# jaak-s/libfastsparse

Measured on AMD Instinct MI355X. Metric: fp64 CSR SpMV effective GB/s (% HBM3E peak), higher is better.
Workload: dtype f64

## Files before the change

### libfastsparse_amd/csrc/fs_common.h

```cpp
#pragma once

#include <hip/hip_runtime.h>
#include <stdint.h>
#include <stdio.h>
#include <mutex>
#include <string>
#include <vector>

#include "fastsparse_hip.h"
#include "fs_geometry.h"

namespace fs {

constexpr int kBlock = 256;
constexpr int kChunk = 2048;
constexpr int kPerThread = kChunk / kBlock;

void set_error(const std::string &msg);
int hip_fail(hipError_t e, const char *what, const char *file, int line);

#define FS_HIP(call)                                                   \
  do {                                                                 \
    hipError_t e_ = (call);                                            \
    if (e_ != hipSuccess) return ::fs::hip_fail(e_, #call, __FILE__, __LINE__); \
// ... 25 lines not shown
  int nrow = 0, ncol = 0;
  int64_t nnz = 0;
  int *row_ptr = nullptr;
  int *cols = nullptr;
  double *vals = nullptr;
  bool owns = true;
  bool released = false, released_valued = false;
  bool has_vals() const { return vals != nullptr || (released && released_valued); }
  int nchunks = 0;
  int *first_row = nullptr;
  double *head = nullptr;
  double *tail = nullptr;
  int spanning = 0;
  TiledCsr *tiled = nullptr;
  TiledCsr *tiledx = nullptr;
  BinnedCsr *binned = nullptr;
  BinnedCsr *binned2 = nullptr, *binned4 = nullptr;
  bool tried2 = false, tried4 = false;
  double *spmm_scratch = nullptr;
  size_t spmm_scratch_doubles = 0;
  signed char spmm_choice[17] = {};
  float candidate_ms[4] = {0.f, 0.f, 0.f, 0.f};
  mutable int max_row_len = -1;
  bool two_pass_clear_win = false;
  float build_ms[8] = {0.f, 0.f, 0.f, 0.f, 0.f, 0.f, 0.f, 0.f};
  struct PartCuts { int n = 0, kind = 0; bool cut = false; std::vector<int> rows, units; };
  std::vector<PartCuts> part_plans;
  PartCuts partk[2];
};

struct TiledCsr {
  bool built = false;
  bool ldsx = false;
  int R = 0, W = 0, P = 0, J = 0, lcol_bits = kTiledColBits;
  float entries_per_tile = 0.f;
  unsigned *pk = nullptr;
  double *vals = nullptr;
  int4 *items = nullptr;
  int *item_ptr = nullptr;
  int nitems = 0;
  int *panel_row = nullptr;
  int split = 0;
  int nvrow = 0;
  int *vfirst = nullptr;
  double *yv = nullptr;
  int slots = 256;
  HostMirror<int> h_panel_row, h_chunk_panel;
  std::vector<int> h_chunk_need;
  int nchunks = 0;
  int *chunk_panel = nullptr;
  int *chunk_item = nullptr;
  bool shared = false;
  bool orderable = false;
  int *chunk_ord = nullptr;
  int *ticket = nullptr;
};


struct LongRows {
  int nlong = 0;
  int64_t n = 0;
  int bcols = kLongBandA;
  int B = 0;
  int *row = nullptr;
  uint16_t *lcol = nullptr;
  uint16_t *lrow = nullptr;
  double *vals = nullptr;
  int64_t *band_ptr = nullptr;
  unsigned *seg_ptr = nullptr;
  double *ylong = nullptr;
  double *ypart = nullptr;
  int nwg = 0;
};

struct BinnedCsr {
  bool built = false;
  LongRows *lr = nullptr;
  int kw = 1;
  int bcols = kBinCols;
  int B = 0, P = 0;
  int64_t n = 0;
  uint16_t *lcol = nullptr;
  double *vals = nullptr;
  unsigned *gdst = nullptr;
  uint16_t *lrow = nullptr;
  uint8_t *lrow8 = nullptr;
  uint16_t *gbase = nullptr;
  int64_t dummies = 0;
  bool lrow_tried = false;
  double *prod = nullptr;
  unsigned *band_ptr = nullptr;
  int nwg1 = 0;
  int slots = 0;
  unsigned *bin_ptr = nullptr;
  int *panel_row = nullptr;
  int split = 0, nvrow = 0;
  int *vfirst = nullptr;
  double *yv = nullptr;
  HostMirror<unsigned> h_band_ptr;
  HostMirror<int> h_panel_row, h_vfirst;
};

struct HostPipe {
  double *sx = nullptr, *sy = nullptr;
  size_t cx = 0, cy = 0;
  hipStream_t stream = nullptr;
  static constexpr int kMaxChunks = 32;
  hipEvent_t ev[kMaxChunks] = {};
  int nev = 0;
};
void free_host_pipe(HostPipe &H);

}

struct fs_matrix_s {
  fs::DeviceCsr a;
  fs::DeviceCsr at;
  bool has_t = false;
  int device = 0;
  std::mutex lock;
  hipStream_t last_stream = nullptr;
  bool last_async = false;
  fs::HostPipe pipe;
};

struct fs_cbcsr_s {
  int nrow = 0, ncol = 0, nblocks = 0, colblocksize = 0;
  int64_t nnz = 0;
  int *row_ptr = nullptr;
  int *cols = nullptr;
  int device = 0;
  fs::DeviceCsr cells;
  double *cell_sums = nullptr;
  bool use_cells = false;
  fs::DeviceCsr rows;
  bool use_rows = false;
  std::mutex lock;
};

namespace fs {

bool roctx_enabled();
void roctx_push(const char *name);
void roctx_pop();
struct Range {
  bool on;
  explicit Range(const char *name) : on(roctx_enabled()) { if (on) roctx_push(name); }
  ~Range() { if (on) roctx_pop(); }
  Range(const Range &) = delete;
  Range &operator=(const Range &) = delete;
};
#define FS_RANGE(name) ::fs::Range fs_range_(name)

struct Options {
  int strict_order = 0;
  int spmv_kernel = 0;
  int tiling = 1;
  int tile_rows = 0;
  int tile_cols = 0;
  int tile_split = 0;
  int tiled_flags = 0;
  int reproducible = 0;
  int bin_wgs = 0;
  int bin_flags = 0;
  int bin_rows = 0;
  int ldsx = 1;
// ... 195 lines not shown
```

### libfastsparse_amd/csrc/fs_copies.hip

```cpp
#include <algorithm>
#include <vector>

#include "fs_format_util.h"
#include "fs_plan.h"

namespace fs {

static_assert(sizeof(WorkItem) == sizeof(int4) && sizeof(RowLen) == sizeof(int2), "fs_plan.h's plain structs are the device's int4 / int2");

__global__ void piece_count_kernel(int nrow, int split, const int *__restrict__ row_ptr, int *__restrict__ cnt)
{
  const int r = blockIdx.x * blockDim.x + threadIdx.x;
  if (r > nrow) return;
  if (r == nrow) { cnt[r] = 0; return; }
  const int len = row_ptr[r + 1] - row_ptr[r];
  cnt[r] = len <= split ? 1 : (len + split - 1) / split;
}

__global__ void vrow_fill_kernel(int nrow, int split, const int *__restrict__ row_ptr, const int *__restrict__ vfirst,
                                 int *__restrict__ vrow_ptr)
{
  const int r = blockIdx.x * blockDim.x + threadIdx.x;
  if (r > nrow) return;
  if (r == nrow) { vrow_ptr[vfirst[nrow]] = row_ptr[nrow]; return; }
// ... 636 lines not shown
  if (mode == 1 && !ldsx && tiled_hopeless(A.nnz, ntiles, P, slots, x_bytes)) return FS_OK;
  if (ntiles >= (1ll << 31)) return FS_OK;
  T->R = R; T->W = W; T->P = P; T->J = J;
  T->entries_per_tile = (float)((double)A.nnz / (double)ntiles);
  FS_HIP(traced_malloc(&T->panel_row, sizeof(int) * panel_row.size()));
  FS_HIP(hipMemcpyAsync(T->panel_row, panel_row.data(), sizeof(int) * panel_row.size(), hipMemcpyHostToDevice, s));

  const size_t n = (size_t)A.nnz;
  Scratch<int> vrows, tile_ptr;
  Scratch<unsigned> keys, skeys, idx_in, idx_out;
  Scratch<char> tmp;
  FS_HIP(vrows.alloc(n));
  FS_HIP(keys.alloc(n));
  FS_HIP(skeys.alloc(n));
  FS_HIP(idx_in.alloc(n));
  FS_HIP(idx_out.alloc(n));
  FS_HIP(tile_ptr.alloc((size_t)ntiles + 1));
  FS_HIP(traced_malloc(&T->pk, sizeof(unsigned) * (n + 8)));
  if (A.vals) FS_HIP(traced_malloc(&T->vals, sizeof(double) * (n + 8)));
  hipLaunchKernelGGL(tile_key_kernel, dim3(grid_for(A.nnz)), dim3(256), 0, s, V.nvrow, A.nnz, P, W, J, V.vrow_ptr, T->panel_row,
                     A.cols, vrows.p, keys.p);
  const unsigned *sorted_keys = nullptr, *perm = nullptr;
  if (int rc = sorted_runs(tmp, keys.p, skeys.p, idx_in.p, idx_out.p, n, ntiles, tile_ptr.p, s, &sorted_keys, &perm)) return rc;
  hipLaunchKernelGGL(tile_pack_kernel, dim3(grid_for(A.nnz)), dim3(256), 0, s, A.nnz, W, J, T->lcol_bits, sorted_keys, perm,
                     vrows.p, T->panel_row, A.cols, A.vals, T->pk, T->vals);
  FS_HIP(hipGetLastError());
  std::vector<int> tp((size_t)ntiles + 1);
  FS_HIP(hipMemcpyAsync(tp.data(), tile_ptr.p, sizeof(int) * tp.size(), hipMemcpyDeviceToHost, s));
  FS_HIP(hipStreamSynchronize(s));
  std::vector<WorkItem> items;
  std::vector<int> item_ptr;
  cut_work_items(tp, P, J, items, item_ptr);
  T->nitems = (int)items.size();
  FS_HIP(traced_malloc(&T->items, sizeof(int4) * (items.size() ? items.size() : 1)));
  FS_HIP(traced_malloc(&T->item_ptr, sizeof(int) * item_ptr.size()));
  if (!items.empty()) FS_HIP(hipMemcpy(T->items, items.data(), sizeof(int4) * items.size(), hipMemcpyHostToDevice));
  FS_HIP(hipMemcpy(T->item_ptr, item_ptr.data(), sizeof(int) * item_ptr.size(), hipMemcpyHostToDevice));
  if (ldsx && T->nitems > 0)
    if (int rc = reorder_ldsx_items(T, s)) return rc;
  if (ldsx) {
    static const bool plain = [] { const char *v = getenv("FS_LDSX_ORDER"); return v && *v == '1'; }();
    std::vector<int> chunk_panel, chunk_item, chunk_ord;
    T->shared = plan_ldsx_chunks(item_ptr, (int64_t)items.size(), P, slots, plain, chunk_panel, chunk_item, chunk_ord);
    if (int rc = upload_ldsx_chunks(T, A.nrow, chunk_panel, chunk_item, chunk_ord)) return rc;
  }
  T->built = true;
  return FS_OK;
}

int build_tiled(DeviceCsr &A, hipStream_t s) { return optional_copy(build_tiled_impl(A, s, A.tiled, false), A.tiled, free_tiled_slot); }

int build_tiledx(DeviceCsr &A, hipStream_t s) { return optional_copy(build_tiled_impl(A, s, A.tiledx, true), A.tiledx, free_tiled_slot); }

__global__ void bin_key_kernel(int nvrow, int64_t nnz, int P, int bcols, const int *__restrict__ vrow_ptr,
                               const int *__restrict__ panel_row, const int *__restrict__ cols,
                               int *__restrict__ vrows, unsigned *__restrict__ keys)
{
  const int64_t i = (int64_t)blockIdx.x * blockDim.x + threadIdx.x;
  if (i >= nnz) return;
  const int v = last_le(vrow_ptr, nvrow, i);
  vrows[i] = v;
  keys[i] = (unsigned)(cols[i] / bcols) * (unsigned)P + (unsigned)last_le(panel_row, P, v);
}

__global__ void bin_groups_kernel(int B, int P, int ge, const int *__restrict__ run_ptr, unsigned *__restrict__ g1,
                                  unsigned *__restrict__ g2, const unsigned *__restrict__ xs = nullptr)
{
  const int64_t k = (int64_t)blockIdx.x * blockDim.x + threadIdx.x;
  const int64_t nruns = (int64_t)B * P;
  if (k > nruns) return;
  if (k == nruns) { g1[k] = 0; g2[k] = 0; return; }
  const int b = (int)(k / P), p = (int)(k % P);
  const unsigned dum = xs ? xs[run_ptr[k + 1]] - xs[run_ptr[k]] : 0u;
  const unsigned g = ((unsigned)(run_ptr[k + 1] - run_ptr[k]) + dum + (unsigned)ge - 1u) / (unsigned)ge;
  g1[k] = g;
  g2[(int64_t)p * B + b] = g;
}

__global__ void bin_scatter_kernel(int64_t nnz, int B, int P, int bcols, int ge, const unsigned *__restrict__ skeys,
                                   const unsigned *__restrict__ perm, const int *__restrict__ vrows,
                                   const int *__restrict__ panel_row, const int *__restrict__ cols,
                                   const double *__restrict__ vals, const int *__restrict__ run_ptr,
                                   const unsigned *__restrict__ start1, const unsigned *__restrict__ start2,
                                   uint16_t *__restrict__ lcol, double *__restrict__ vals2, uint16_t *__restrict__ lrow)
{
  const int64_t i = (int64_t)blockIdx.x * blockDim.x + threadIdx.x;
  if (i >= nnz) return;
  const unsigned key = skeys[i], src = perm[i];
  const int b = (int)(key / (unsigned)P), p = (int)(key % (unsigned)P);
  const int64_t rank = i - run_ptr[key];
  const int64_t pos1 = (int64_t)start1[key] * ge + rank;
  const int64_t pos2 = (int64_t)start2[(int64_t)p * B + b] * ge + rank;
  lcol[pos1] = (uint16_t)(cols[src] - b * bcols);
  if (vals) vals2[pos2] = vals[src];
  lrow[pos2] = (uint16_t)(vrows[src] - panel_row[p]);
}

__global__ void bin_gap_kernel(int64_t nnz, int P, const unsigned *__restrict__ skeys, const unsigned *__restrict__ perm,
                               const int *__restrict__ vrows, const int *__restrict__ run_ptr, unsigned *__restrict__ extra)
{
  const int64_t i = (int64_t)blockIdx.x * blockDim.x + threadIdx.x;
  if (i > nnz) return;
  if (i == nnz) { extra[i] = 0; return; }
  const unsigned key = skeys[i];
  unsigned e = 0;
  if (i > run_ptr[key]) {
    const int gap = vrows[perm[i]] - vrows[perm[i - 1]];
    if (gap > 255) e = (unsigned)(gap - 1) / 255u;
  }
  extra[i] = e;
}

__global__ void bin_scatter8_kernel(int64_t nnz, int B, int P, int bcols, int ge, const unsigned *__restrict__ skeys,
                                    const unsigned *__restrict__ perm, const int *__restrict__ vrows,
                                    const int *__restrict__ panel_row, const int *__restrict__ cols,
                                    const double *__restrict__ vals, const int *__restrict__ run_ptr,
                                    const unsigned *__restrict__ xs, const unsigned *__restrict__ start1,
                                    const unsigned *__restrict__ start2, uint16_t *__restrict__ lcol, double *__restrict__ vals2,
                                    uint8_t *__restrict__ lrow8, uint16_t *__restrict__ gbase)
{
  const int64_t i = (int64_t)blockIdx.x * blockDim.x + threadIdx.x;
  if (i >= nnz) return;
  const unsigned key = skeys[i], src = perm[i];
  const int b = (int)(key / (unsigned)P), p = (int)(key % (unsigned)P);
  const int64_t first = run_ptr[key];
  const unsigned dum = xs[i + 1] - xs[i];
  const int64_t slot = (i - first) + (int64_t)(xs[i] - xs[first]) + dum;
  const int64_t base1 = (int64_t)start1[key] * ge, base2 = (int64_t)start2[(int64_t)p * B + b] * ge;
  const int row = vrows[src] - panel_row[p];
  const int prev = i > first ? vrows[perm[i - 1]] - panel_row[p] : row;
  for (unsigned m = 0; m < dum; ++m) {
    const int64_t sl = slot - dum + m;
    lrow8[base2 + sl] = 255;
    if ((sl & (ge - 1)) == 0) gbase[(base2 + sl) / ge] = (uint16_t)(prev + 255 * (int)m);
  }
  const int before = prev + 255 * (int)dum;
  lcol[base1 + slot] = (uint16_t)(cols[src] - b * bcols);
  if (vals) vals2[base2 + slot] = vals[src];
  lrow8[base2 + slot] = (uint8_t)(row - before);
  if ((slot & (ge - 1)) == 0) gbase[(base2 + slot) / ge] = (uint16_t)before;
}

__global__ void bin_gdst_kernel(int B, int P, const unsigned *__restrict__ start1, const unsigned *__restrict__ start2,
                                unsigned *__restrict__ gdst)
{
  const int64_t k = (int64_t)blockIdx.x * blockDim.x + threadIdx.x;
  if (k >= (int64_t)B * P) return;
  const int b = (int)(k / P), p = (int)(k % P);
  const unsigned a = start1[k], n = start1[k + 1] - a, d = start2[(int64_t)p * B + b];
  for (unsigned j = 0; j < n; ++j) gdst[a + j] = d + j;
}

__global__ void bin_ptr_kernel(int B, int P, const unsigned *__restrict__ start1, const unsigned *__restrict__ start2,
                               unsigned *__restrict__ band_ptr, unsigned *__restrict__ bin_ptr)
{
  const int64_t k = (int64_t)blockIdx.x * blockDim.x + threadIdx.x;
  if (k <= B) band_ptr[k] = start1[k * P];
  if (k <= P) bin_ptr[k] = start2[k * B];
}

__global__ void long_candidates_kernel(int nrow, int minlen, const int *__restrict__ row_ptr, int *__restrict__ count, int cap,
                                       int2 *__restrict__ out)
{
  const int r = blockIdx.x * blockDim.x + threadIdx.x;
  if (r >= nrow) return;
  const int len = row_ptr[r + 1] - row_ptr[r];
  if (len < minlen) return;
  const int k = atomicAdd(count, 1);
  if (k < cap) out[k] = make_int2(r, len);
}

__global__ void long_mark_kernel(int nlong, const int *__restrict__ rows, int *__restrict__ row_to_long)
{
  const int i = blockIdx.x * blockDim.x + threadIdx.x;
  if (i < nlong) row_to_long[rows[i]] = i;
}

// ... 197 lines not shown
  N->split = V.split;
  N->nvrow = V.nvrow;
  const int nvrow = V.nvrow;

  std::vector<int> vp;
  if (int rc = V.fetch(vp, s)) return rc;
  static const double fill = [] { const char *v = getenv("FS_BIN_FILL"); return v && *v ? atof(v) / 100.0 : 0.8; }();
  static const int min_panels = [] { const char *v = getenv("FS_BIN_MIN_PANELS"); return v && *v ? atoi(v) : 1; }();
  const std::vector<int> panel_row = plan_two_pass_panels(vp, nvrow, A.nnz, g.R, slots, fill, min_panels, kw);
  const int P = (int)panel_row.size() - 1;
  const int B = (A.ncol + bcols - 1) / bcols;
  const int64_t nruns = (int64_t)P * B;
  if (nruns >= (1ll << 28)) return FS_OK;
  if (o.binning == 1 && two_pass_padding_dominates(A.nnz, nruns, ge)) return FS_OK;
  N->P = P; N->B = B; N->slots = slots;
  FS_HIP(traced_malloc(&N->panel_row, sizeof(int) * panel_row.size()));
  FS_HIP(hipMemcpyAsync(N->panel_row, panel_row.data(), sizeof(int) * panel_row.size(), hipMemcpyHostToDevice, s));

  const size_t n = (size_t)A.nnz;
  Scratch<int> vrows, run_ptr;
  Scratch<unsigned> keys, skeys, idx_in, idx_out, g1, g2, start1, start2;
  Scratch<char> tmp, tmp2;
  FS_HIP(vrows.alloc(n));
  FS_HIP(keys.alloc(n));
  FS_HIP(skeys.alloc(n));
  FS_HIP(idx_in.alloc(n));
  FS_HIP(idx_out.alloc(n));
  FS_HIP(run_ptr.alloc((size_t)nruns + 1));
  FS_HIP(g1.alloc((size_t)nruns + 1));
  FS_HIP(g2.alloc((size_t)nruns + 1));
  FS_HIP(start1.alloc((size_t)nruns + 1));
  FS_HIP(start2.alloc((size_t)nruns + 1));
  FS_HIP(traced_malloc(&N->band_ptr, sizeof(unsigned) * ((size_t)B + 1)));
  FS_HIP(traced_malloc(&N->bin_ptr, sizeof(unsigned) * ((size_t)P + 1)));
  hipLaunchKernelGGL(bin_key_kernel, dim3(grid_for(A.nnz)), dim3(256), 0, s, nvrow, A.nnz, P, bcols, V.vrow_ptr, N->panel_row,
                     A.cols, vrows.p, keys.p);
  const unsigned *sorted_keys = nullptr, *perm = nullptr;
  if (int rc = sorted_runs(tmp, keys.p, skeys.p, idx_in.p, idx_out.p, n, nruns, run_ptr.p, s, &sorted_keys, &perm)) return rc;
  Scratch<unsigned> extra, xs;
  Scratch<char> tmp3;
  bool rows8 = false;
  int64_t dummies = 0;
  if (kw == 1 && bcols == kBinCols && !(o.bin_flags & 64) && A.nnz > 0) {
    FS_HIP(extra.alloc(n + 1));
    FS_HIP(xs.alloc(n + 1));
    hipLaunchKernelGGL(bin_gap_kernel, dim3(grid_for(A.nnz + 1)), dim3(256), 0, s, A.nnz, P, sorted_keys, perm, vrows.p, run_ptr.p, extra.p);
    FS_HIP(hipGetLastError());
    if (int rc = device_exclusive_scan(tmp3, extra.p, xs.p, n + 1, s)) return rc;
    unsigned total = 0;
    if (int rc = read_back(&total, (const unsigned *)xs.p + n, s)) return rc;
    dummies = total;
    rows8 = (o.bin_flags & 128) || (double)total <= 0.01 * (double)A.nnz;
  }
  hipLaunchKernelGGL(bin_groups_kernel, dim3(grid_for(nruns + 1)), dim3(256), 0, s, B, P, ge, run_ptr.p, g1.p, g2.p,
                     rows8 ? (const unsigned *)xs.p : (const unsigned *)nullptr);
  FS_HIP(hipGetLastError());
  if (int rc = device_exclusive_scan(tmp2, g1.p, start1.p, (size_t)nruns + 1, s)) return rc;
  if (int rc = device_exclusive_scan(tmp2, g2.p, start2.p, (size_t)nruns + 1, s)) return rc;
  hipLaunchKernelGGL(bin_ptr_kernel, dim3(grid_for((B > P ? B : P) + 1)), dim3(256), 0, s, B, P, start1.p, start2.p, N->band_ptr,
                     N->bin_ptr);
  FS_HIP(hipGetLastError());
  unsigned total_groups = 0;
  if (int rc = read_back(&total_groups, (const unsigned *)N->band_ptr + B, s)) return rc;
  const int64_t groups = total_groups;
  if (groups >= (1ll << 28) * (int64_t)kw) return FS_OK;
  if (groups >= (1ll << 32) - 1) return FS_OK;
  N->n = groups * ge;
  if (o.binning == 1 && kw == 1 && two_pass_hopeless(N->n, A.vals != nullptr, B, ncu, bcols, nvrow, A.ncol, A.nnz)) return FS_OK;

  const size_t np = (size_t)N->n;
  FS_HIP(traced_malloc(&N->lcol, sizeof(uint16_t) * np));
  if (rows8) {
    FS_HIP(traced_malloc(&N->lrow8, np));
    FS_HIP(traced_malloc(&N->gbase, sizeof(uint16_t) * (size_t)(groups ? groups : 1)));
    N->dummies = dummies;
  } else {
    FS_HIP(traced_malloc(&N->lrow, sizeof(uint16_t) * np));
  }
  FS_HIP(traced_malloc(&N->gdst, sizeof(unsigned) * (size_t)groups));
  FS_HIP(traced_malloc(&N->prod, sizeof(double) * np * (size_t)kw));
  if (A.vals) {
    FS_HIP(traced_malloc(&N->vals, sizeof(double) * np));
    FS_HIP(hipMemsetAsync(N->vals, 0, sizeof(double) * np, s));
  }
  FS_HIP(hipMemsetD16Async((hipDeviceptr_t)N->lcol, (unsigned short)bcols, np, s));
  if (rows8) {
    FS_HIP(hipMemsetAsync(N->lrow8, 0, np, s));
    FS_HIP(hipMemsetAsync(N->gbase, 0, sizeof(uint16_t) * (size_t)(groups ? groups : 1), s));
    hipLaunchKernelGGL(bin_scatter8_kernel, dim3(grid_for(A.nnz)), dim3(256), 0, s, A.nnz, B, P, bcols, ge, sorted_keys, perm, vrows.p,
                       N->panel_row, A.cols, A.vals, run_ptr.p, xs.p, start1.p, start2.p, N->lcol, N->vals, N->lrow8, N->gbase);
  } else {
    FS_HIP(hipMemsetAsync(N->lrow, 0, sizeof(uint16_t) * np, s));
    hipLaunchKernelGGL(bin_scatter_kernel, dim3(grid_for(A.nnz)), dim3(256), 0, s, A.nnz, B, P, bcols, ge, sorted_keys, perm, vrows.p,
                       N->panel_row, A.cols, A.vals, run_ptr.p, start1.p, start2.p, N->lcol, N->vals, N->lrow);
  }
  hipLaunchKernelGGL(bin_gdst_kernel, dim3(grid_for(nruns)), dim3(256), 0, s, B, P, start1.p, start2.p, N->gdst);
  FS_HIP(hipGetLastError());

  {
    const int64_t by_size = (N->n * kw + kBinShareMin - 1) / kBinShareMin;
    N->nwg1 = (int)(by_size < ncu ? by_size : ncu);
  }
  FS_HIP(hipStreamSynchronize(s));
  N->built = true;
  return FS_OK;
}

int build_binned(DeviceCsr &A, hipStream_t s)
{
  LongRows *lr = nullptr;
  Scratch<int> main_rp, main_cols;
  Scratch<double> main_vals;
  int64_t main_nnz = 0;
  if (split_long_rows(A, s, &lr, main_rp, main_cols, main_vals, &main_nnz) != FS_OK) {
    free_long_rows(lr);
    (void)hipGetLastError();
  }
  int rc;
  if (lr) {
    DeviceCsr M;
    M.nrow = A.nrow; M.ncol = A.ncol; M.nnz = main_nnz;
    M.row_ptr = main_rp.p; M.cols = main_cols.p; M.vals = A.vals ? main_vals.p : nullptr; M.owns = false;
    rc = build_binned_impl(M, s, A.binned, 1);
    if (rc == FS_OK && A.binned && A.binned->built) { A.binned->lr = lr; lr = nullptr; }
    M = DeviceCsr();
  } else {
    rc = build_binned_impl(A, s, A.binned, 1);
  }
  free_long_rows(lr);
  return optional_copy(rc, A.binned, free_binned_slot);
}

int build_binned_k(DeviceCsr &A, int kw, hipStream_t s)
{
  if (kw != 2 && kw != 4) return FS_ERR_ARG;
  BinnedCsr *&slot = kw == 2 ? A.binned2 : A.binned4;
  (kw == 2 ? A.tried2 : A.tried4) = true;
  return optional_copy(build_binned_impl(A, s, slot, kw), slot, free_binned_slot);
}

constexpr double kTiledBestEntriesPerMs = 152e6;

template <typename F>
static int time_product(F launch, hipStream_t s, hipEvent_t e0, hipEvent_t e1, float *median, int reps = 5)
{
  float t[5] = {1e30f, 1e30f, 1e30f, 1e30f, 1e30f};
  for (int rep = -1; rep < reps; ++rep) {
    FS_HIP(hipEventRecord(e0, s));
    if (int rc = launch()) return rc;
    FS_HIP(hipEventRecord(e1, s));
    FS_HIP(hipEventSynchronize(e1));
    float ms = 0.f;
    FS_HIP(hipEventElapsedTime(&ms, e0, e1));
    if (rep >= 0) t[rep] = ms;
  }
  std::sort(t, t + reps);
  *median = t[reps / 2];
  return FS_OK;
}

int two_pass_clear_win(DeviceCsr &A, hipStream_t s, bool *win)
{
  *win = false;
  const Options &o = options();
  if (!(A.binned && A.binned->built) || o.binning != 1 || o.tiling != 1 || A.nnz < (32ll << 20) || 8.0 * (double)A.ncol <= (double)(4 << 20)) return FS_OK;
  Scratch<double> x, y;
  if (x.alloc((size_t)A.ncol) != hipSuccess || y.alloc((size_t)A.nrow) != hipSuccess) { (void)hipGetLastError(); return FS_OK; }
  FS_HIP(hipMemsetAsync(x, 0, sizeof(double) * (size_t)A.ncol, s));
  hipEvent_t e0, e1;
  FS_HIP(hipEventCreate(&e0));
  if (hipEventCreate(&e1) != hipSuccess) { (void)hipEventDestroy(e0); return FS_OK; }
  float t = 1e30f;
  const int rc = time_product([&] { return launch_spmv_binned(A, y, x, s); }, s, e0, e1, &t, 2);
  (void)hipEventDestroy(e0);
  (void)hipEventDestroy(e1);
  if (rc != FS_OK) return rc;
  *win = (double)t <= (double)A.nnz / (A.vals ? kTiledBestEntriesPerMs : 200e6);
// ... 53 lines not shown
```

### libfastsparse_amd/csrc/fs_kernels_twopass.hip

```cpp
#include <stdlib.h>

#include "fs_kernel_util.h"

namespace fs {


template <int U, bool NTLD, bool NTST, int BC>
__device__ __forceinline__ void expand_share(double *__restrict__ xband, int ncol, int B, const unsigned *__restrict__ band_ptr,
                                             const uint16_t *__restrict__ lcol, const unsigned *__restrict__ gdst,
                                             const double *__restrict__ x, int xs, double *__restrict__ prod, unsigned g0,
                                             unsigned g1)
{
  const int t = threadIdx.x;
  if (g0 >= g1) return;
  int b;
  {
    int lo = 0, hi = B - 1;
    while (lo < hi) {
      const int mid = lo + ((hi - lo + 1) >> 1);
      if (band_ptr[mid] <= g0) lo = mid; else hi = mid - 1;
    }
    b = lo;
  }
  for (unsigned g = g0; g < g1; ++b) {
// ... 301 lines not shown
      const int w = (ncol - c0 < BC) ? ncol - c0 : BC;
      if (have != b) request(b);
      __syncthreads();
#pragma unroll
      for (int j = 0; j < BC / kBinBlock; ++j) {
        const int i = j * kBinBlock + t;
        xband[i] = (i < w) ? rn[j] : 0.0;
      }
      if (t < 8) xband[BC + t] = 0.0;
      __syncthreads();
      if (b + 1 < B && eb < e_end) request(b + 1);
      if (ORDERED) {
        const int64_t s0 = band_ptr[b] + seg_ptr[b * (kLongOwners + 1) + wave], s1 = band_ptr[b] + seg_ptr[b * (kLongOwners + 1) + wave + 1];
        const int64_t lo = s0 > e ? s0 : e, hi = s1 < eb ? s1 : eb;
        for (int64_t o0 = lo; o0 < hi; o0 += 128) {
          const int64_t o = o0 + 2 * lane;
          const bool live = o < hi;
          wave_step(o, live, live ? o : lo);
        }
      } else {
        for (int64_t o0 = e; o0 < eb; o0 += 2 * kBinBlock) {
          const int64_t o = o0 + 2 * t;
          const bool live = o < eb;
          wave_step(o, live, live ? o : e);
        }
      }
      e = eb;
    }
  }
  __syncthreads();
  if (ORDERED) {
    double *__restrict__ mine = ypart + (int64_t)blockIdx.x * nlong;
    for (int i = t; i < nlong; i += kBinBlock) mine[i] = acc[i];
  } else {
    for (int i = t; i < nlong; i += kBinBlock) {
      const double v = acc[i];
      if (v != 0.0) unsafeAtomicAdd(ylong + i, v);
    }
  }
}

__global__ __launch_bounds__(kBlock) void longrows_combine_kernel(int nlong, int nwg, const double *__restrict__ ypart, double *__restrict__ ylong)
{
  const int i = blockIdx.x * kBlock + threadIdx.x;
  if (i >= nlong) return;
  double acc = 0.0;
  for (int w = 0; w < nwg; ++w) acc += ypart[(int64_t)w * nlong + i];
  ylong[i] = acc;
}

__global__ __launch_bounds__(kBlock) void longrows_scatter_kernel(int nlong, const int *__restrict__ row, const double *__restrict__ ylong,
                                                                 double *__restrict__ y, int ys, int row0, int row1)
{
  const int i = blockIdx.x * kBlock + threadIdx.x;
  if (i >= nlong) return;
  const int r = row[i];
  if (r >= row0 && r < row1) y[(int64_t)r * ys] = 0.0 + ylong[i];
}

static int launch_longrows(const DeviceCsr &A, const LongRows &L, const double *x, int xs, hipStream_t s)
{
  const bool ordered = reproducible_now();
  if (!ordered || L.n == 0 || L.nwg == 0)
    if (int rc = launch_zero(L.ylong, sizeof(double) * (size_t)L.nlong, s)) return rc;
  if (L.n == 0 || L.nwg == 0) return FS_OK;
#define FS_LONG(V, BC, NA, ORD)                                                                                              \
  hipLaunchKernelGGL((spmv_longrows_kernel<V, BC, NA, ORD>), dim3(L.nwg), dim3(kBinBlock), 0, s, A.ncol, L.B, L.nlong, L.band_ptr, \
                     L.seg_ptr, L.lcol, L.lrow, L.vals, x, xs, L.ylong, L.ypart)
#define FS_LONG2(V, BC, NA) do { if (ordered) FS_LONG(V, BC, NA, true); else FS_LONG(V, BC, NA, false); } while (0)
  if (L.bcols == kLongBandB) { if (A.has_vals()) FS_LONG2(true, kLongBandB, kLongRowsB); else FS_LONG2(false, kLongBandB, kLongRowsB); }
  else                       { if (A.has_vals()) FS_LONG2(true, kLongBandA, kLongRowsA); else FS_LONG2(false, kLongBandA, kLongRowsA); }
#undef FS_LONG2
#undef FS_LONG
  FS_HIP(hipGetLastError());
  if (ordered) {
    hipLaunchKernelGGL(longrows_combine_kernel, dim3((unsigned)((L.nlong + kBlock - 1) / kBlock)), dim3(kBlock), 0, s, L.nlong, L.nwg, L.ypart,
                       L.ylong);
    FS_HIP(hipGetLastError());
  }
  return FS_OK;
}


template <int K, int U>
__global__ __launch_bounds__(kBinBlock) void spmm_expand_kernel(
    int ncol, int B, const unsigned *__restrict__ band_ptr, const uint16_t *__restrict__ lcol,
    const unsigned *__restrict__ gdst, const double *__restrict__ X, int xs, double *__restrict__ prod)
{
  constexpr int BC = kBinCols / K;
  constexpr int GE = kBinGroup / K;
  constexpr int LP = K / 2;
  constexpr int EPS = kBinBlock / LP;
  __shared__ __attribute__((aligned(16))) double xband[kBinCols + 8];
  const int t = threadIdx.x;
  const int le = t / LP, h = t % LP;
  const uint64_t groups = band_ptr[B];
  const unsigned g0 = (unsigned)(groups * blockIdx.x / gridDim.x), g1 = (unsigned)(groups * (blockIdx.x + 1) / gridDim.x);
  if (g0 >= g1) return;
  int b;
  {
    int lo = 0, hi = B - 1;
    while (lo < hi) {
      const int mid = lo + ((hi - lo + 1) >> 1);
      if (band_ptr[mid] <= g0) lo = mid; else hi = mid - 1;
    }
    b = lo;
  }
  for (unsigned g = g0; g < g1; ++b) {
    const unsigned gb = band_ptr[b + 1] < g1 ? band_ptr[b + 1] : g1;
    if (gb <= g) continue;
    const int c0 = b * BC;
    const int w = (ncol - c0 < BC) ? ncol - c0 : BC;
    __syncthreads();
    {
      double r[kBinCols / kBinBlock];
#pragma unroll
      for (int j = 0; j < kBinCols / kBinBlock; ++j) {
        const int f = j * kBinBlock + t, i = f / K, q = f % K;
        r[j] = __builtin_nontemporal_load(X + (int64_t)(c0 + (i < w ? i : w - 1)) * xs + q);
      }
#pragma unroll
      for (int j = 0; j < kBinCols / kBinBlock; ++j) {
        const int f = j * kBinBlock + t;
        xband[f] = (f / K < w) ? r[j] : 0.0;
      }
      if (t < 8) xband[kBinCols + t] = 0.0;
    }
    __syncthreads();
    const int64_t e0 = (int64_t)g * GE, e1 = (int64_t)gb * GE;
    constexpr int64_t kRound = (int64_t)U * EPS;
    int64_t o = e0 + le;
    for (; o - le + kRound <= e1; o += kRound) {
      unsigned a[U], d[U];
#pragma unroll
      for (int k = 0; k < U; ++k) {
        const int64_t e = o + (int64_t)k * EPS;
        a[k] = lcol[e];
        d[k] = gdst[e / GE];
      }
      __builtin_amdgcn_sched_barrier(0);
#pragma unroll
      for (int k = 0; k < U; ++k) {
        const int64_t e = o + (int64_t)k * EPS;
        const v2d p = *reinterpret_cast<const v2d *>(&xband[a[k] * K + 2 * h]);
        __builtin_nontemporal_store(p, (v2d *)(prod + ((int64_t)d[k] * GE + (e % GE)) * K + 2 * h));
      }
    }
    for (; o < e1; o += EPS) {
      const unsigned a = lcol[o];
      const unsigned d = gdst[o / GE];
      const v2d p = *reinterpret_cast<const v2d *>(&xband[a * K + 2 * h]);
      __builtin_nontemporal_store(p, (v2d *)(prod + ((int64_t)d * GE + (o % GE)) * K + 2 * h));
    }
    g = gb;
  }
}

template <bool VALUED, int K>
__global__ __launch_bounds__(kBinBlock) void spmm_reduce_kernel(
    const unsigned *__restrict__ bin_ptr_all, const int *__restrict__ panel_row_all, const uint16_t *__restrict__ lrow,
    const double *__restrict__ vals, const double *__restrict__ prod, double *__restrict__ Y, int ys, int pbase)
{
  const unsigned *__restrict__ bin_ptr = bin_ptr_all + pbase;
  const int *__restrict__ panel_row = panel_row_all + pbase;
  constexpr int GE = kBinGroup / K;
  constexpr int EPL = 8 / K;
  __shared__ double ytile[kBinRowsMax];
  const int t = threadIdx.x;
  const int r0 = panel_row[blockIdx.x], nr = panel_row[blockIdx.x + 1] - r0;
  for (int i = t; i < nr * K; i += kBinBlock) ytile[i] = 0.0;
  __syncthreads();
  const int64_t e0 = (int64_t)bin_ptr[blockIdx.x] * GE, e1 = (int64_t)bin_ptr[blockIdx.x + 1] * GE;
  typedef uint16_t rows_t __attribute__((ext_vector_type(EPL)));
  typedef double vals_t __attribute__((ext_vector_type(EPL)));
#define FS_ADD(idx, val) __hip_atomic_fetch_add(&ytile[idx], val, __ATOMIC_RELAXED, __HIP_MEMORY_SCOPE_WORKGROUP)
  auto add8 = [&](const rows_t a, const v2d (&p)[4], const vals_t v) {
#pragma unroll
    for (int q = 0; q < EPL; ++q) {
      const int base = (int)a[q] * K;
#pragma unroll
      for (int j = 0; j < K; j += 2) {
        v2d t2 = p[(q * K + j) / 2];
        if (VALUED) { t2.x *= v[q]; t2.y *= v[q]; }
        FS_ADD(base + j, t2.x);
        FS_ADD(base + j + 1, t2.y);
      }
    }
  };
  constexpr int64_t kStep = (int64_t)EPL * kBinBlock;
  constexpr int64_t kRound = 2 * kStep;
  int64_t e = e0 + (int64_t)EPL * t;
  for (; e - EPL * t + kRound <= e1; e += kRound) {
    rows_t a[2];
    v2d p[2][4];
    vals_t v[2] = {};
#pragma unroll
    for (int k = 0; k < 2; ++k) {
      const int64_t ek = e + k * kStep;
      a[k] = *reinterpret_cast<const rows_t *>(lrow + ek);
      if (VALUED) v[k] = *reinterpret_cast<const vals_t *>(vals + ek);
#pragma unroll
      for (int j = 0; j < 4; ++j) p[k][j] = *reinterpret_cast<const v2d *>(prod + ek * K + 2 * j);
    }
    __builtin_amdgcn_sched_barrier(0);
    add8(a[0], p[0], v[0]);
    add8(a[1], p[1], v[1]);
  }
  for (; e < e1; e += kStep) {
    const rows_t a = *reinterpret_cast<const rows_t *>(lrow + e);
    vals_t v = {};
    if (VALUED) v = *reinterpret_cast<const vals_t *>(vals + e);
    v2d p[4];
#pragma unroll
    for (int j = 0; j < 4; ++j) p[j] = *reinterpret_cast<const v2d *>(prod + e * K + 2 * j);
    add8(a, p, v);
  }
#undef FS_ADD
  __syncthreads();
  for (int i = t; i < nr * K; i += kBinBlock) Y[(int64_t)(r0 + i / K) * ys + (i % K)] = ytile[i];
}

template <bool VALUED, int K, int DEPTH>
__global__ __launch_bounds__(64) void spmm_reduce_ordered_kernel(
    const unsigned *__restrict__ bin_ptr_all, const int *__restrict__ panel_row_all, const uint16_t *__restrict__ lrow,
    const double *__restrict__ vals, const double *__restrict__ prod, double *__restrict__ Y, int ys, int pbase)
{
  const unsigned *__restrict__ bin_ptr = bin_ptr_all + pbase;
  const int *__restrict__ panel_row = panel_row_all + pbase;
  constexpr int GE = kBinGroup / K;
  constexpr int EPL = 8 / K;
  __shared__ double ytile[kBinRowsMax];
  const int t = threadIdx.x;
  const int r0 = panel_row[blockIdx.x], nr = panel_row[blockIdx.x + 1] - r0;
  for (int i = t; i < nr * K; i += 64) ytile[i] = 0.0;
  const int64_t e0 = (int64_t)bin_ptr[blockIdx.x] * GE, e1 = (int64_t)bin_ptr[blockIdx.x + 1] * GE;
  typedef uint16_t rows_t __attribute__((ext_vector_type(EPL)));
  typedef double vals_t __attribute__((ext_vector_type(EPL)));
#define FS_ADD(idx, val) __hip_atomic_fetch_add(&ytile[idx], val, __ATOMIC_RELAXED, __HIP_MEMORY_SCOPE_WORKGROUP)
  auto add8 = [&](const rows_t a, const v2d (&p)[4], const vals_t v) {
#pragma unroll
    for (int q = 0; q < EPL; ++q) {
      const int base = (int)a[q] * K;
#pragma unroll
      for (int j = 0; j < K; j += 2) {
        v2d t2 = p[(q * K + j) / 2];
        if (VALUED) { t2.x *= v[q]; t2.y *= v[q]; }
        FS_ADD(base + j, t2.x);
        FS_ADD(base + j + 1, t2.y);
      }
    }
  };
  constexpr int64_t kStep = (int64_t)EPL * 64;
  rows_t a[DEPTH];
  v2d p[DEPTH][4];
  vals_t v[VALUED ? DEPTH : 1] = {};
  auto fetch = [&](int k, int64_t e) {
    const int64_t ec = (e + EPL <= e1) ? e : (e1 - e0 >= EPL ? e1 - EPL : e0);
    a[k] = *reinterpret_cast<const rows_t *>(lrow + ec);
    if (VALUED) v[k] = *reinterpret_cast<const vals_t *>(vals + ec);
#pragma unroll
    for (int j = 0; j < 4; ++j) p[k][j] = *reinterpret_cast<const v2d *>(prod + ec * K + 2 * j);
  };
  if (e1 > e0) {
    int64_t e = e0 + (int64_t)EPL * t;
#pragma unroll
    for (int k = 0; k < DEPTH; ++k) fetch(k, e + (int64_t)k * kStep);
    for (; e - EPL * t < e1; e += (int64_t)DEPTH * kStep) {
#pragma unroll
      for (int k = 0; k < DEPTH; ++k) {
        const int64_t ek = e + (int64_t)k * kStep;
        const rows_t ak = a[k];
        const v2d pk[4] = {p[k][0], p[k][1], p[k][2], p[k][3]};
        const vals_t vk = v[VALUED ? k : 0];
        fetch(k, ek + (int64_t)DEPTH * kStep);
        if (ek + EPL <= e1) add8(ak, pk, vk);
      }
    }
  }
#undef FS_ADD
  __syncthreads();
  for (int i = t; i < nr * K; i += 64) Y[(int64_t)(r0 + i / K) * ys + (i % K)] = ytile[i];
}

template <int K>
__global__ __launch_bounds__(kBlock) void tiled_combine_k_kernel(int nrow, const int *__restrict__ vfirst,
                                                                const double *__restrict__ yv, double *__restrict__ Y, int ys,
                                                                int row0 = 0)
{
  const int64_t i = (int64_t)row0 * K + (int64_t)blockIdx.x * kBlock + threadIdx.x;
  const int64_t r = i / K;
  const int j = (int)(i % K);
  if (r >= nrow) return;
  const int a = vfirst[r], b = vfirst[r + 1];
  double acc = yv[(int64_t)a * K + j];
  for (int v = a + 1; v < b; ++v) acc += yv[(int64_t)v * K + j];
  Y[r * ys + j] = acc;
}

// ... 62 lines not shown
    const int flags = options().bin_flags;
#define FS_EXPAND4(U)                                                                                       \
  do {                                                                                                      \
    if (flags & 16) { if (flags & 8) FS_EXPAND(U, true, false);  else FS_EXPAND(U, true, true); }           \
    else            { if (flags & 8) FS_EXPAND(U, false, false); else FS_EXPAND(U, false, true); }          \
  } while (0)
#define FS_EXPAND(U, NL, NS)                                                                                      \
  hipLaunchKernelGGL((spmv_expand_kernel<U, NL, NS>), dim3(nwg1), dim3(kBinBlock), 0, s, A.ncol, N.B, N.band_ptr, \
                     N.lcol, N.gdst, x, xs, N.prod, 0u, (unsigned)(N.n >> kBinGroupLog))
    if (N.bcols == kBinColsBig)
      hipLaunchKernelGGL((spmv_expand_kernel<4, false, true, kBinColsBig>), dim3(nwg1), dim3(kBinBlock), 0, s, A.ncol, N.B,
                         N.band_ptr, N.lcol, N.gdst, x, xs, N.prod, 0u, (unsigned)(N.n >> kBinGroupLog));
    else if ((flags & 3) == 1) FS_EXPAND4(8);
    else if ((flags & 3) == 2) FS_EXPAND4(2);
    else                       FS_EXPAND4(4);
#undef FS_EXPAND4
#undef FS_EXPAND
    FS_HIP(hipGetLastError());
  }
  if (N.lr && p0 == 0)
    if (int rc = launch_longrows(A, *N.lr, x, xs, s)) return rc;
  if (p1 > p0) {
    const bool ordered = reproducible_now() || (options().bin_flags & 32);
    if (ordered && N.lrow8 && !N.lrow) ensure_two_byte_ids(*A.binned, s);
#define FS_ORDERED(RM, L8)                                                                                                     \
  do {                                                                                                                         \
    if (N.vals)                                                                                                                \
      hipLaunchKernelGGL((spmv_reduce_ordered_kernel<true, false, RM, FS_ORDERED_DEPTH_VALUED, L8>), dim3(p1 - p0), dim3(64), 0, s, \
                         N.bin_ptr, N.panel_row, N.lrow, N.vals, N.prod, out, os, p0, N.lrow8, N.gbase);                       \
    else                                                                                                                       \
      hipLaunchKernelGGL((spmv_reduce_ordered_kernel<false, false, RM, FS_ORDERED_DEPTH, L8>), dim3(p1 - p0), dim3(64), 0, s,  \
                         N.bin_ptr, N.panel_row, N.lrow, N.vals, N.prod, out, os, p0, N.lrow8, N.gbase);                       \
  } while (0)
    if (N.bcols == kBinColsBig && ordered)  FS_ORDERED(kBinRowsBig, false);
    else if (ordered && N.lrow8 && !N.lrow) FS_ORDERED(kBinRowsMax, true);
    else if (ordered)                       FS_ORDERED(kBinRowsMax, false);
    else
      launch_reduce(N, out, os, p0, p1, options().bin_flags, s);
#undef FS_ORDERED
    FS_HIP(hipGetLastError());
  }
  if (N.split && row1 > row0) {
    if (int rc = launch_tiled_combine(row1, N.vfirst, N.yv, y, ys, row0, s)) return rc;
  }
  if (N.lr && row1 > row0) {
    hipLaunchKernelGGL(longrows_scatter_kernel, dim3((unsigned)((N.lr->nlong + kBlock - 1) / kBlock)), dim3(kBlock), 0, s, N.lr->nlong,
                       N.lr->row, N.lr->ylong, y, ys, row0, row1);
    FS_HIP(hipGetLastError());
  }
  return FS_OK;
}

int launch_expand_groups(const DeviceCsr &A, const double *x, unsigned g0, unsigned g1, int wgs, hipStream_t s)
{
  const BinnedCsr &N = *A.binned;
  if (g1 <= g0 || wgs <= 0) return FS_OK;
#define FS_XH(BC)                                                                                                         \
  hipLaunchKernelGGL((spmv_expand_kernel<4, false, true, BC>), dim3(wgs), dim3(kBinBlock), 0, s, A.ncol, N.B, N.band_ptr, \
                     N.lcol, N.gdst, x, 1, N.prod, g0, g1)
  if (N.bcols == kBinColsBig) FS_XH(kBinColsBig);
  else                        FS_XH(kBinCols);
#undef FS_XH
  FS_HIP(hipGetLastError());
  return FS_OK;
}

int launch_reduce_panels(const DeviceCsr &A, double *y, int p0, int p1, hipStream_t s)
{
  const BinnedCsr &N = *A.binned;
  if (p1 <= p0) return FS_OK;
  launch_reduce(N, y, 1, p0, p1, 0, s);
  FS_HIP(hipGetLastError());
  return FS_OK;
}

int launch_spmm_binned(const DeviceCsr &A, const BinnedCsr &N, double *Y, const double *X, hipStream_t s, int xs, int ys, int p0,
                       int p1, int row0, int row1)
{
  const int K = N.kw;
  double *out = N.split ? N.yv : Y;
  const int os = N.split ? K : ys;
  if (p1 < 0) { p0 = 0; p1 = N.P; row0 = 0; row1 = A.nrow; }
  const int nwg1 = (p0 != 0) ? 0 : ((options().bin_wgs > 0 && options().bin_wgs < N.nwg1) ? options().bin_wgs : N.nwg1);
#define FS_XP(KK)                                                                                                  \
  hipLaunchKernelGGL((spmm_expand_kernel<KK, 4>), dim3(nwg1), dim3(kBinBlock), 0, s, A.ncol, N.B, N.band_ptr, N.lcol, \
                     N.gdst, X, xs, N.prod)
  if (nwg1 > 0) {
    if (K == 2) FS_XP(2); else FS_XP(4);
    FS_HIP(hipGetLastError());
  }
#undef FS_XP
  if (p1 > p0) {
    const bool ordered = reproducible_now() || (options().bin_flags & 32);
#define FS_RP(V, KK)                                                                                                            \
  do {                                                                                                                          \
    if (ordered)                                                                                                                \
      hipLaunchKernelGGL((spmm_reduce_ordered_kernel<V, KK, (V && KK == 2) ? 12 : FS_ORDERED_DEPTH>), dim3(p1 - p0), dim3(64), 0, s, N.bin_ptr, \
                         N.panel_row, N.lrow, N.vals, N.prod, out, os, p0);                                                     \
    else                                                                                                                        \
      hipLaunchKernelGGL((spmm_reduce_kernel<V, KK>), dim3(p1 - p0), dim3(kBinBlock), 0, s, N.bin_ptr, N.panel_row, N.lrow,     \
                         N.vals, N.prod, out, os, p0);                                                                          \
  } while (0)
    if (K == 2) { if (N.vals) FS_RP(true, 2); else FS_RP(false, 2); }
    else        { if (N.vals) FS_RP(true, 4); else FS_RP(false, 4); }
#undef FS_RP
    FS_HIP(hipGetLastError());
  }
  if (N.split && row1 > row0) {
    const unsigned grid = (unsigned)(((int64_t)(row1 - row0) * K + kBlock - 1) / kBlock);
    if (K == 2)
      hipLaunchKernelGGL(tiled_combine_k_kernel<2>, dim3(grid), dim3(kBlock), 0, s, row1, N.vfirst, N.yv, Y, ys, row0);
    else
      hipLaunchKernelGGL(tiled_combine_k_kernel<4>, dim3(grid), dim3(kBlock), 0, s, row1, N.vfirst, N.yv, Y, ys, row0);
    FS_HIP(hipGetLastError());
  }
  return FS_OK;
}

}
```

Baseline: 2688.

## Move value multiply into expand pass for K=4 binned SpMM and add specialized reduce

For four-column binned SpMM, matrix values are now stored in pass-1 (column) order. The expand kernel multiplies each gathered X pair by its value before writing the product. This lets a new reduce kernel accumulate the products directly, with no value stream and with optional nontemporal loads. The value read moves into the gather pass and the reduce pass gets lighter. The 8-bit row scatter path was not updated to place values in pass-1 order, so that layout may be inconsistent. The change mainly targets the multi-vector path, not single-vector SpMV.

```diff
diff --git a/libfastsparse_amd/csrc/fs_common.h b/libfastsparse_amd/csrc/fs_common.h
--- a/libfastsparse_amd/csrc/fs_common.h
+++ b/libfastsparse_amd/csrc/fs_common.h
@@ -131,6 +131,7 @@
   int64_t n = 0;
   uint16_t *lcol = nullptr;
   double *vals = nullptr;
+  bool vals_in_pass1 = false;
   unsigned *gdst = nullptr;
   uint16_t *lrow = nullptr;
   uint8_t *lrow8 = nullptr;
diff --git a/libfastsparse_amd/csrc/fs_copies.hip b/libfastsparse_amd/csrc/fs_copies.hip
--- a/libfastsparse_amd/csrc/fs_copies.hip
+++ b/libfastsparse_amd/csrc/fs_copies.hip
@@ -742,7 +742,8 @@
                                    const int *__restrict__ panel_row, const int *__restrict__ cols,
                                    const double *__restrict__ vals, const int *__restrict__ run_ptr,
                                    const unsigned *__restrict__ start1, const unsigned *__restrict__ start2,
-                                   uint16_t *__restrict__ lcol, double *__restrict__ vals2, uint16_t *__restrict__ lrow)
+                                   uint16_t *__restrict__ lcol, double *__restrict__ vals2, uint16_t *__restrict__ lrow,
+                                   bool vals_in_pass1)
 {
   const int64_t i = (int64_t)blockIdx.x * blockDim.x + threadIdx.x;
   if (i >= nnz) return;
@@ -752,7 +753,7 @@
   const int64_t pos1 = (int64_t)start1[key] * ge + rank;
   const int64_t pos2 = (int64_t)start2[(int64_t)p * B + b] * ge + rank;
   lcol[pos1] = (uint16_t)(cols[src] - b * bcols);
-  if (vals) vals2[pos2] = vals[src];
+  if (vals) vals2[vals_in_pass1 ? pos1 : pos2] = vals[src];
   lrow[pos2] = (uint16_t)(vrows[src] - panel_row[p]);
 }
 
@@ -1116,6 +1117,7 @@
   if (A.vals) {
     FS_HIP(traced_malloc(&N->vals, sizeof(double) * np));
     FS_HIP(hipMemsetAsync(N->vals, 0, sizeof(double) * np, s));
+    N->vals_in_pass1 = kw == 4;
   }
   FS_HIP(hipMemsetD16Async((hipDeviceptr_t)N->lcol, (unsigned short)bcols, np, s));
   if (rows8) {
@@ -1126,7 +1128,7 @@
   } else {
     FS_HIP(hipMemsetAsync(N->lrow, 0, sizeof(uint16_t) * np, s));
     hipLaunchKernelGGL(bin_scatter_kernel, dim3(grid_for(A.nnz)), dim3(256), 0, s, A.nnz, B, P, bcols, ge, sorted_keys, perm, vrows.p,
-                       N->panel_row, A.cols, A.vals, run_ptr.p, start1.p, start2.p, N->lcol, N->vals, N->lrow);
+                       N->panel_row, A.cols, A.vals, run_ptr.p, start1.p, start2.p, N->lcol, N->vals, N->lrow, N->vals_in_pass1);
   }
   hipLaunchKernelGGL(bin_gdst_kernel, dim3(grid_for(nruns)), dim3(256), 0, s, B, P, start1.p, start2.p, N->gdst);
   FS_HIP(hipGetLastError());
diff --git a/libfastsparse_amd/csrc/fs_kernels_twopass.hip b/libfastsparse_amd/csrc/fs_kernels_twopass.hip
--- a/libfastsparse_amd/csrc/fs_kernels_twopass.hip
+++ b/libfastsparse_amd/csrc/fs_kernels_twopass.hip
@@ -407,10 +407,11 @@
 }
 
 
-template <int K, int U>
+template <int K, int U, bool VALUED = false>
 __global__ __launch_bounds__(kBinBlock) void spmm_expand_kernel(
     int ncol, int B, const unsigned *__restrict__ band_ptr, const uint16_t *__restrict__ lcol,
-    const unsigned *__restrict__ gdst, const double *__restrict__ X, int xs, double *__restrict__ prod)
+    const unsigned *__restrict__ gdst, const double *__restrict__ vals, const double *__restrict__ X, int xs,
+    double *__restrict__ prod)
 {
   constexpr int BC = kBinCols / K;
   constexpr int GE = kBinGroup / K;
@@ -457,24 +458,28 @@
     int64_t o = e0 + le;
     for (; o - le + kRound <= e1; o += kRound) {
       unsigned a[U], d[U];
+      double v[VALUED ? U : 1];
 #pragma unroll
       for (int k = 0; k < U; ++k) {
         const int64_t e = o + (int64_t)k * EPS;
         a[k] = lcol[e];
         d[k] = gdst[e / GE];
+        if (VALUED) v[k] = vals[e];
       }
       __builtin_amdgcn_sched_barrier(0);
 #pragma unroll
       for (int k = 0; k < U; ++k) {
         const int64_t e = o + (int64_t)k * EPS;
-        const v2d p = *reinterpret_cast<const v2d *>(&xband[a[k] * K + 2 * h]);
+        v2d p = *reinterpret_cast<const v2d *>(&xband[a[k] * K + 2 * h]);
+        if (VALUED) { p.x *= v[k]; p.y *= v[k]; }
         __builtin_nontemporal_store(p, (v2d *)(prod + ((int64_t)d[k] * GE + (e % GE)) * K + 2 * h));
       }
     }
     for (; o < e1; o += EPS) {
       const unsigned a = lcol[o];
       const unsigned d = gdst[o / GE];
-      const v2d p = *reinterpret_cast<const v2d *>(&xband[a * K + 2 * h]);
+      v2d p = *reinterpret_cast<const v2d *>(&xband[a * K + 2 * h]);
+      if (VALUED) { const double v = vals[o]; p.x *= v; p.y *= v; }
       __builtin_nontemporal_store(p, (v2d *)(prod + ((int64_t)d * GE + (o % GE)) * K + 2 * h));
     }
     g = gb;
@@ -539,6 +544,68 @@
 #pragma unroll
     for (int j = 0; j < 4; ++j) p[j] = *reinterpret_cast<const v2d *>(prod + e * K + 2 * j);
     add8(a, p, v);
+  }
+#undef FS_ADD
+  __syncthreads();
+  for (int i = t; i < nr * K; i += kBinBlock) Y[(int64_t)(r0 + i / K) * ys + (i % K)] = ytile[i];
+}
+
+template <bool NTLD>
+__global__ __launch_bounds__(kBinBlock) void spmm_reduce4_kernel(
+    const unsigned *__restrict__ bin_ptr_all, const int *__restrict__ panel_row_all, const uint16_t *__restrict__ lrow,
+    const double *__restrict__ prod, double *__restrict__ Y, int ys, int pbase)
+{
+  constexpr int K = 4;
+  const unsigned *__restrict__ bin_ptr = bin_ptr_all + pbase;
+  const int *__restrict__ panel_row = panel_row_all + pbase;
+  __shared__ double ytile[kBinRowsMax];
+  const int t = threadIdx.x;
+  const int r0 = panel_row[blockIdx.x], nr = panel_row[blockIdx.x + 1] - r0;
+  for (int i = t; i < nr * K; i += kBinBlock) ytile[i] = 0.0;
+  __syncthreads();
+  const int64_t q0 = (int64_t)bin_ptr[blockIdx.x] * kBinGroup, q1 = (int64_t)bin_ptr[blockIdx.x + 1] * kBinGroup;
+#define FS_ADD(idx, val) __hip_atomic_fetch_add(&ytile[idx], val, __ATOMIC_RELAXED, __HIP_MEMORY_SCOPE_WORKGROUP)
+  constexpr int64_t kStep = 8 * kBinBlock, kRound = 2 * kStep;
+  const int wave0 = (t >> 6) * 512, lane0 = wave0 + 2 * (t & 63);
+  const int h2 = 2 * (t & 1);
+  int64_t qb = q0;
+  for (; qb + kRound <= q1; qb += kRound) {
+    const int64_t q = qb + lane0;
+    unsigned a[2][4];
+    v2d p[2][4];
+#pragma unroll
+    for (int k = 0; k < 2; ++k)
+#pragma unroll
+      for (int j = 0; j < 4; ++j) {
+        const int64_t qk = q + k * kStep + 128 * j;
+        a[k][j] = lrow[qk / K];
+        p[k][j] = stream_load<NTLD>((const v2d *)(prod + qk));
+      }
+    __builtin_amdgcn_sched_barrier(0);
+#pragma unroll
+    for (int k = 0; k < 2; ++k)
+#pragma unroll
+      for (int j = 0; j < 4; ++j) {
+        const int base = (int)a[k][j] * K + h2;
+        FS_ADD(base, p[k][j].x);
+        FS_ADD(base + 1, p[k][j].y);
+      }
+  }
+  for (; qb + wave0 < q1; qb += kStep) {
+    const int64_t q = qb + lane0;
+    unsigned a[4];
+    v2d p[4];
+#pragma unroll
+    for (int j = 0; j < 4; ++j) {
+      const int64_t qj = q + 128 * j, qc = qj < q1 ? qj : q1 - 2;
+      a[j] = lrow[qc / K];
+      p[j] = stream_load<NTLD>((const v2d *)(prod + qc));
+    }
+#pragma unroll
+    for (int j = 0; j < 4; ++j) {
+      const int base = (int)a[j] * K + h2;
+      if (q + 128 * j < q1) { FS_ADD(base, p[j].x); FS_ADD(base + 1, p[j].y); }
+    }
   }
 #undef FS_ADD
   __syncthreads();
@@ -767,27 +834,35 @@
   const int os = N.split ? K : ys;
   if (p1 < 0) { p0 = 0; p1 = N.P; row0 = 0; row1 = A.nrow; }
   const int nwg1 = (p0 != 0) ? 0 : ((options().bin_wgs > 0 && options().bin_wgs < N.nwg1) ? options().bin_wgs : N.nwg1);
-#define FS_XP(KK)                                                                                                  \
-  hipLaunchKernelGGL((spmm_expand_kernel<KK, 4>), dim3(nwg1), dim3(kBinBlock), 0, s, A.ncol, N.B, N.band_ptr, N.lcol, \
-                     N.gdst, X, xs, N.prod)
+#define FS_XP(KK, V)                                                                                                  \
+  hipLaunchKernelGGL((spmm_expand_kernel<KK, 4, V>), dim3(nwg1), dim3(kBinBlock), 0, s, A.ncol, N.B, N.band_ptr, N.lcol, \
+                     N.gdst, N.vals, X, xs, N.prod)
   if (nwg1 > 0) {
-    if (K == 2) FS_XP(2); else FS_XP(4);
+    if (K == 2) FS_XP(2, false); else if (N.vals && N.vals_in_pass1) FS_XP(4, true); else FS_XP(4, false);
     FS_HIP(hipGetLastError());
   }
 #undef FS_XP
   if (p1 > p0) {
     const bool ordered = reproducible_now() || (options().bin_flags & 32);
+    const bool plain = (options().bin_flags & 256) != 0;
+    if (K == 4 && N.vals && !N.vals_in_pass1) return FS_ERR_ARG;
 #define FS_RP(V, KK)                                                                                                            \
   do {                                                                                                                          \
     if (ordered)                                                                                                                \
       hipLaunchKernelGGL((spmm_reduce_ordered_kernel<V, KK, (V && KK == 2) ? 12 : FS_ORDERED_DEPTH>), dim3(p1 - p0), dim3(64), 0, s, N.bin_ptr, \
                          N.panel_row, N.lrow, N.vals, N.prod, out, os, p0);                                                     \
+    else if (KK == 2)                                                                                                           \
+      hipLaunchKernelGGL((spmm_reduce_kernel<V, 2>), dim3(p1 - p0), dim3(kBinBlock), 0, s, N.bin_ptr, N.panel_row, N.lrow,      \
+                         N.vals, N.prod, out, os, p0);                                                                          \
+    else if (plain)                                                                                                             \
+      hipLaunchKernelGGL((spmm_reduce4_kernel<false>), dim3(p1 - p0), dim3(kBinBlock), 0, s, N.bin_ptr, N.panel_row, N.lrow,    \
+                         N.prod, out, os, p0);                                                                                  \
     else                                                                                                                        \
-      hipLaunchKernelGGL((spmm_reduce_kernel<V, KK>), dim3(p1 - p0), dim3(kBinBlock), 0, s, N.bin_ptr, N.panel_row, N.lrow,     \
-                         N.vals, N.prod, out, os, p0);                                                                          \
+      hipLaunchKernelGGL((spmm_reduce4_kernel<true>), dim3(p1 - p0), dim3(kBinBlock), 0, s, N.bin_ptr, N.panel_row, N.lrow,     \
+                         N.prod, out, os, p0);                                                                                  \
   } while (0)
     if (K == 2) { if (N.vals) FS_RP(true, 2); else FS_RP(false, 2); }
-    else        { if (N.vals) FS_RP(true, 4); else FS_RP(false, 4); }
+    else        FS_RP(false, 4);
 #undef FS_RP
     FS_HIP(hipGetLastError());
   }
```

After: 2644. 0.983x the previous value.
